# mathcom/G2Vec

Hardware: NVIDIA H100
Metric: cbow_context_windows_per_sec (higher is better)
Workload: dtype f32

## Files before the change

g2vec_b200/_capi.py:

```python
import ctypes
import os

from . import build as _build

_lib = None

_vp, _i32, _i64, _u32, _u64, _f32 = (ctypes.c_void_p, ctypes.c_int32, ctypes.c_int64, ctypes.c_uint32,
                                     ctypes.c_uint64, ctypes.c_float)

SIGNATURES = {
    "g2v_abi_version": (ctypes.c_int, []),
    "g2v_last_error": (ctypes.c_char_p, []),
    "g2v_device_info": (ctypes.c_int, [_vp, _vp, _vp, _vp]),
    "g2v_launch_count": (_i64, []),
    "g2v_walk_workspace_bytes": (ctypes.c_size_t, []),
    "g2v_walk_launch": (ctypes.c_int, [_vp, _vp, _vp, _i32, _i64, _i32, _u64, _u32, _i64, _i64, _i64,
                                       _vp, _vp, _vp, _vp]),
    "g2v_walk_packed_bytes": (ctypes.c_int, [_i32, _i64, _vp, _vp]),
    "g2v_walk_prepare": (ctypes.c_int, [_vp, _vp, _vp, _i32, _i64, _vp, _vp, _vp, _vp, _vp]),
    "g2v_walk_launch_packed": (ctypes.c_int, [_vp, _vp, _i32, _i32, _i64, _i32, _u64, _u32, _i64, _i64, _i64,
                                              _vp, _vp, _vp, _vp, _vp]),
    "g2v_walk_host": (ctypes.c_int, [_vp, _vp, _vp, _i32, _i64, _i32, _u64, _u32, _i64, _i64, _i64, _vp, _vp]),
    "g2v_cbow_fwdbwd": (ctypes.c_int, [_vp, _vp, _vp, _vp, _i64, _i64, _f32, _vp, _vp, _vp, _vp, _vp, _vp,
                                       _i32, _i32, _i32, _vp]),
    "g2v_cbow_fwdbwd_csc": (ctypes.c_int, [_vp, _vp, _vp, _vp, _i64, _f32, _vp, _vp, _vp, _vp, _vp, _vp, _vp, _vp,
                                           _vp, _i32, _i32, _i32, _vp]),
    "g2v_cbow_fwd_do": (ctypes.c_int, [_vp, _vp, _vp, _vp, _i64, _f32, _vp, _vp, _vp, _vp, _vp, _vp, _i32, _i32, _i32,
                                       _vp]),
    "g2v_cbow_lazy_adam": (ctypes.c_int, [_vp, _vp, _vp, _vp, _i64, _vp, _vp, _vp, _vp, _vp, _vp, _vp, _i32, _i32, _f32,
                                          _f32, _f32, _f32, _i32, _vp, _vp]),
    "g2v_cbow_det_workspace_bytes": (ctypes.c_size_t, [_i64, _i32]),
    "g2v_cbow_fwdbwd_csc_det": (ctypes.c_int, [_vp, _vp, _vp, _vp, _i64, _f32, _vp, _vp, _vp, _vp, _vp, _vp, _vp, _vp,
                                               _vp, _i32, _i32, _i32, _vp, _i32, _vp]),
    "g2v_cbow_fwd_do_det": (ctypes.c_int, [_vp, _vp, _vp, _vp, _i64, _f32, _vp, _vp, _vp, _vp, _vp, _vp, _i32, _i32,
                                           _i32, _vp, _i32, _vp]),
    "g2v_cbow_loop_tail_det": (ctypes.c_int, [_vp, _vp, _vp, _vp, _vp, _i64, _f32, _vp, _vp, _vp, _vp, _vp, _i32, _i32,
                                              _i32, _vp, _i32, _vp]),
    "g2v_cbow_batch_expand": (ctypes.c_int, [_vp, _vp, _vp, _vp, _i64, _vp, _vp, _i32, _i32, _i32, _vp]),
    "g2v_cbow_epoch_order": (ctypes.c_int, [_vp, _i64, _u64, _i32, _i64, _i64, _vp, _vp]),
    "g2v_cbow_batch_plan_workspace_bytes": (ctypes.c_size_t, [_i64, _i64, _i64, _i32]),
    "g2v_cbow_batch_plan": (ctypes.c_int, [_vp, _vp, _vp, _i64, _i64, _i64, _i32, _vp, _vp, _vp, _vp, _vp, _vp]),
    "g2v_cbow_update": (ctypes.c_int, [_vp, _vp, _vp, _vp, _vp, _vp, _vp, _vp, _i32, _i32, _i32, _f32, _f32,
                                       _f32, _f32, _i32, _vp, _vp]),
    "g2v_cbow_update_nvl": (ctypes.c_int, [_vp, _vp, _vp, _vp, _vp, _vp, _i64, _i32, _i32, _i32, _f32, _f32, _f32,
                                           _f32, _i32, _vp, _vp]),
    "g2v_cbow_adam_tick": (ctypes.c_int, [_vp, _f32, _f32, _f32, _vp]),
    "g2v_cbow_eval": (ctypes.c_int, [_vp, _vp, _vp, _vp, _i64, _i64, _vp, _vp, _vp, _i32, _i32, _i32, _vp]),
    "g2v_cbow_loop_init": (ctypes.c_int, [_vp, _i64, _i32, _vp]),
    "g2v_cbow_loop_attach": (ctypes.c_int, [_vp]),
    "g2v_cbow_loop_begin": (ctypes.c_int, [_vp, _vp, _vp, _vp, _i64, _vp]),
    "g2v_cbow_loop_tail": (ctypes.c_int, [_vp, _vp, _vp, _vp, _vp, _i64, _f32, _vp, _vp, _vp, _vp, _vp, _i32, _i32, _i32,
                                          _vp]),
    "g2v_cbow_loop_decide": (ctypes.c_int, [_vp, _vp, _vp, _vp]),
    "g2v_cbow_loop_decide_best": (ctypes.c_int, [_vp, _vp, _vp, _vp, _vp]),
    "g2v_cbow_loop_keep_best": (ctypes.c_int, [_vp, _vp, _vp, _i64, _vp]),
    "g2v_cbow_loop_counters_nvl": (ctypes.c_int, [_vp, _vp, _vp, _vp, _i32, _vp]),
    "g2v_cbow_slab_plan": (ctypes.c_int, [_i32, _i32, _vp]),
    "g2v_cbow_slab_workspace_bytes": (ctypes.c_size_t, [_i64, _i32, _i32]),
    "g2v_cbow_slab_setup": (ctypes.c_int, [_vp, _vp, _vp, _i64, _i64, _i32, _i32, _vp, _vp]),
    "g2v_cbow_fwdbwd_slabs": (ctypes.c_int, [_vp, _vp, _vp, _i64, _i64, _f32, _vp, _vp, _vp, _vp, _vp, _vp,
                                             _i32, _i32, _i32, _i32, _vp, _vp]),
    "g2v_cbow_eval_slabs": (ctypes.c_int, [_vp, _vp, _vp, _i64, _i64, _vp, _vp, _vp, _i32, _i32, _i32, _i32, _vp, _vp]),
    "g2v_cbow_step_host": (ctypes.c_int, [_vp, _vp, _vp, _i64, _i64, _vp, _vp, _vp, _vp, _vp, _vp, _i32, _i32,
                                          _i32, _i32, _f32, _f32, _f32, _f32, _i32, _vp, _vp]),
    "g2v_cbow_r1_prepare": (ctypes.c_int, [_vp, _vp, _vp, _i32, _i32, _vp]),
    "g2v_cbow_r1_windows": (ctypes.c_int, [_vp, _vp, _vp, _vp, _i64, _i64, _f32, _vp, _vp, _vp, _vp, _i32, _i32, _vp]),
    "g2v_cbow_r1_windows_csc": (ctypes.c_int, [_vp, _vp, _vp, _vp, _i64, _f32, _vp, _vp, _vp, _vp, _vp, _vp, _vp,
                                              _i32, _i32, _vp]),
    "g2v_cbow_r1_scratch_bytes": (ctypes.c_size_t, [_i32]),
    "g2v_cbow_r1_update": (ctypes.c_int, [_vp, _vp, _vp, _vp, _vp, _vp, _vp, _vp, _vp, _i32, _i32, _i32, _f32, _f32,
                                         _f32, _f32, _i32, _vp, _vp]),
    "g2v_pcc_zscore": (ctypes.c_int, [_vp, _i32, _i32, _vp, _vp]),
    "g2v_pcc_edge_weights": (ctypes.c_int, [_vp, _i32, _i32, _vp, _vp, _i64, _vp, _vp]),
    "g2v_paths_canonicalise": (ctypes.c_int, [_vp, _i64, _i32, _vp, _vp, _vp]),
    "g2v_paths_mark": (ctypes.c_int, [_vp, _vp, _vp, _vp, _i64, _i32, _vp, _vp]),
    "g2v_paths_set_workspace_bytes": (ctypes.c_size_t, [_i64]),
    "g2v_paths_set_select": (ctypes.c_int, [_vp, _vp, _vp, _vp, _i64, _i32, _vp, _vp, _vp, _vp]),
    "g2v_paths_set_emit": (ctypes.c_int, [_vp, _vp, _vp, _vp, _i64, _i32, _i32, _vp, _i64, _i64, _vp, _vp, _vp, _vp,
                                          _vp, _vp]),
    "g2v_test_l2_rows": (ctypes.c_int, [_vp, _vp, _vp, _i64, _i32, _i32, _vp, _vp]),
# ... 45 lines not shown
```

g2vec_b200/cbow.py:

```python
import math
import time

import numpy as np
import torch

from . import _capi


def split_indices(n, seed):
    perm = np.arange(n, dtype=np.int64)
    np.random.RandomState(seed).shuffle(perm)
    pivot = int(n * 0.8)
    return perm[:pivot], perm[pivot:]


def truncated_normal(shape, stddev, rng):
    x = rng.standard_normal(size=shape)
    bad = np.abs(x) > 2.0
    while bad.any():
        x[bad] = rng.standard_normal(size=int(bad.sum()))
        bad = np.abs(x) > 2.0
    return (x * stddev).astype(np.float32)


# ... 25 lines not shown
        self.device = dev

        def to(a, dt):
            if isinstance(a, torch.Tensor):
                return a.to(device=dev, dtype=dt).contiguous()
            return torch.from_numpy(np.ascontiguousarray(a)).to(device=dev, dtype=dt)

        self.rowptr = to(rowptr, torch.int32)
        self.gene = to(gene, torch.int32)
        self.label = to(label, torch.uint8)
        self.V, self.D = int(n_genes), int(hidden)
        n_flat = self.V * self.D + self.D
        self.nvl = None
        self.lazy = optimizer == "lazy_adam"
        self.det = bool(deterministic)
        self._det_ws = None
        self._lists, self._pending, self._dO = {}, None, None
        if algo == "rows" and nvl_group is not None:
            self.nvl = _nvl_setup(nvl_group, n_flat, dev)
        if algo == "rows":
            self.w_flat = self.nvl["w"] if self.nvl else torch.empty(n_flat, dtype=torch.float32, device=dev)
            self.W_ih = self.w_flat[:self.V * self.D].view(self.V, self.D)
            self.W_ho = self.w_flat[self.V * self.D:]
            self.W_ih.copy_(to(W_ih0, torch.float32).reshape(self.V, self.D))
            self.W_ho.copy_(to(W_ho0, torch.float32).reshape(self.D))
        else:
            self.W_ih = to(W_ih0, torch.float32).reshape(self.V, self.D).clone()
            self.W_ho = to(W_ho0, torch.float32).reshape(self.D).clone()
        self.opt = {"adam": _capi.OPT_ADAM_TF1, "sgd": _capi.OPT_SGD, "lazy_adam": _capi.OPT_ADAM_TF1}[optimizer]
        self.reduce = {"sum": _capi.REDUCE_SUM, "mean": _capi.REDUCE_MEAN}[reduce]
        self.lr, self.beta1, self.beta2, self.eps = float(lr), float(beta1), float(beta2), float(eps)
        z = lambda *s: torch.zeros(*s, dtype=torch.float32, device=dev)
        self.algo = algo
        if self.lazy:
            self.g_ih, self.g_ho = None, z(self.D)
            self.g_flat = self.g_ho
            self.s = self.c = None
        elif algo == "rows":
            self.g_flat = self.nvl["g"].zero_() if self.nvl else z(n_flat)
            self.g_ih = self.g_flat[:self.V * self.D].view(self.V, self.D)
            self.g_ho = self.g_flat[self.V * self.D:]
            self.s = self.c = None
        else:
            self.g_ih = None
            self.g_ho = z(int(self.lib.g2v_cbow_r1_scratch_bytes(self.D)) // 4)
            self.s, self.c = z(self.V), z(self.V)
        self.m_flat = self.v_flat = None
        if self.opt == _capi.OPT_ADAM_TF1 and algo == "rows":
            self.m_flat, self.v_flat = z(n_flat), z(n_flat)
            vd = self.V * self.D
            self.m_ih, self.v_ih = self.m_flat[:vd].view(self.V, self.D), self.v_flat[:vd].view(self.V, self.D)
            self.m_ho, self.v_ho = self.m_flat[vd:], self.v_flat[vd:]
        elif self.opt == _capi.OPT_ADAM_TF1:
            self.m_ih, self.v_ih, self.m_ho, self.v_ho = z(self.V, self.D), z(self.V, self.D), z(self.D), z(self.D)
        else:
            self.m_ih = self.v_ih = self.m_ho = self.v_ho = None
        self.acc = torch.zeros(6, dtype=torch.int64, device=dev)
        self.t = 0
        self.hyper = torch.tensor([1.0, 1.0, 0.0, 0.0], dtype=torch.float32, device=dev)
        if algo == "rank1":
            self._launch("g2v_cbow_r1_prepare", self.W_ih.data_ptr(), self.W_ho.data_ptr(), self.s.data_ptr(), self.V,
                         self.D)

    def _launch(self, name, *args):
        rc = getattr(self.lib, name)(*args, self._stream())
        if rc:
# ... 184 lines not shown
        if self.algo == "rank1":
            self._launch("g2v_cbow_r1_update", self.W_ih.data_ptr(), self.W_ho.data_ptr(), self._ptr(self.m_ih),
                         self._ptr(self.v_ih), self._ptr(self.m_ho), self._ptr(self.v_ho), self.c.data_ptr(),
                         self.g_ho.data_ptr(), self.s.data_ptr(), self.V, self.D, self.opt, self.lr, self.beta1,
                         self.beta2, self.eps, self.t, adev)
            return
        if self.nvl:
            nv = self.nvl
            nv["hg"].barrier(channel=0)
            self._launch("g2v_cbow_update_nvl", nv["hg"].buffer_ptrs_dev, nv["hw"].buffer_ptrs_dev, nv["g_mc"],
                         nv["w_mc"], self._ptr(self.m_flat), self._ptr(self.v_flat), self.V * self.D + self.D,
                         nv["rank"], nv["world"], self.opt, self.lr, self.beta1, self.beta2, self.eps, self.t, adev)
            nv["hg"].barrier(channel=1)
            return
        self._launch("g2v_cbow_update", self.W_ih.data_ptr(), self.W_ho.data_ptr(), self._ptr(self.m_ih),
                     self._ptr(self.v_ih), self._ptr(self.m_ho), self._ptr(self.v_ho), self.g_ih.data_ptr(),
                     self.g_ho.data_ptr(), self.V, self.D, self.opt, self.lr, self.beta1, self.beta2, self.eps, self.t,
                     adev)

    def evaluate(self, win, slot, win_begin=0, n_win=None):
        lo = int(win_begin)
        n = int((win.shape[0] - win_begin) if n_win is None else n_win)
        rec = self.prepared(win)
        r = choose_route(self.algo, False, False, rec, lo, n)
        acc = self.acc.data_ptr() + 8 * slot
        if r in ("r1", "r1_csc"):
            self._launch("g2v_cbow_r1_windows", self.rowptr.data_ptr(), self.gene.data_ptr(), self.label.data_ptr(),
                         self._ptr(win), lo, n, 0.0, self.s.data_ptr(), 0, 0, acc, self.V, self.reduce)
        elif r == "slabs":
            self._launch("g2v_cbow_eval_slabs", self.gene.data_ptr(), self.label.data_ptr(), self._ptr(win), lo, n,
                         self.W_ih.data_ptr(), self.W_ho.data_ptr(), acc, self.V, self.D, self.reduce, self._n_slabs,
                         rec.slabs[(lo, n)].data_ptr())
        else:
            self._launch("g2v_cbow_eval", self.rowptr.data_ptr(), self.gene.data_ptr(), self.label.data_ptr(),
                         self._ptr(win), lo, n, self.W_ih.data_ptr(), self.W_ho.data_ptr(), acc, self.V, self.D,
                         self.reduce)

    def loss_sum(self, acc_host):
        return float(acc_host[:1].view(torch.float64)[0])


def check_config(algo, optimizer, deterministic, several_gpus=False, batch=0, reshuffle=False, patience=1):
    if isinstance(patience, bool) or not isinstance(patience, (int, np.integer)) or patience < 1:
        raise ValueError("patience must be an int >= 1 (the number of bad epochs in a row that stops the run)")
    if algo not in ("rows", "rank1"):
        raise ValueError("algo must be 'rows' (gather/scatter of embedding rows) or 'rank1' (collapsed)")
    if reshuffle and batch <= 0:
        raise ValueError("reshuffle=True needs mini-batches (batch > 0)")
    if deterministic and several_gpus:
        raise ValueError("deterministic=True runs on one GPU only")
    if deterministic and algo == "rank1" and batch > 0:
        raise ValueError("deterministic=True with algo='rank1' needs a full batch: rank1's mini-batch c uses atomics")
    if optimizer == "lazy_adam" and algo != "rows":
        raise ValueError("optimizer='lazy_adam' needs algo='rows' (rank1 keeps s = W_ih.W_ho, which every W_ho step "
                         "changes for every gene)")
    if optimizer == "lazy_adam" and several_gpus:
        raise ValueError("optimizer='lazy_adam' runs on one GPU only")


class _WindowList:

    def __init__(self, win, n):
        self.win, self.n = win, n
        self.cscptr = self.pos = self.dO = None
        self.slabs = {}
        self.plan, self.B, self.brp = None, 0, None

    def whole(self, win_begin, n):
        return self.cscptr is not None and win_begin == 0 and n == self.n
# ... 503 lines not shown
```

g2vec_b200/csrc/g2v_cbow.cu:

```cuda
#include "g2v_cbow_common.cuh"

namespace g2v {

constexpr int kRowsEval = 0, kRowsScatter = 1, kRowsCsc = 2;

template <int VEC, int MODE>
__global__ void __launch_bounds__(kCbowWarps * 32)
cbow_rows_kernel(const int32_t *__restrict__ rowptr, const int32_t *__restrict__ gene,
                 const uint8_t *__restrict__ label, const int32_t *__restrict__ win,
                 int64_t win_begin, int64_t n_win, float inv_n, const float *__restrict__ W_ih,
                 const float *__restrict__ W_ho, float *__restrict__ g_ih, float *__restrict__ g_ho,
                 double *__restrict__ loss_sum, unsigned long long *__restrict__ n_correct,
                 int32_t reduce_mean, const int32_t *__restrict__ skip, float *__restrict__ dO_pos,
                 const int32_t *__restrict__ carried) {
    G2V_SKIP_IF_STOPPED(skip);
    G2V_SKIP_IF_STOPPED(carried);
    constexpr bool BACKWARD = MODE != kRowsEval;
    constexpr int D = 128 * VEC;
    constexpr int D4 = D / 4;
    constexpr int UNR = 8 / VEC;
    __shared__ float sh_gho[BACKWARD ? D : 1];
    __shared__ CtaAcc sh_acc;
    const int lane = threadIdx.x & 31, warp = threadIdx.x >> 5;
    if (BACKWARD) for (int i = threadIdx.x; i < D; i += blockDim.x) sh_gho[i] = 0.f;
    if (threadIdx.x == 0) { sh_acc.loss = 0.0; sh_acc.correct = 0ull; }
    __syncthreads();

    const float4 *__restrict__ W4 = reinterpret_cast<const float4 *>(W_ih);
    float4 who[VEC], gho[VEC];
#pragma unroll
    for (int v = 0; v < VEC; ++v) {
        who[v] = ldg4(reinterpret_cast<const float4 *>(W_ho) + v * 32 + lane);
        gho[v] = make_float4(0.f, 0.f, 0.f, 0.f);
    }
    unsigned correct_acc = 0;
    float loss_acc = 0.f;

    const int64_t warps_total = (int64_t)gridDim.x * kCbowWarps;
    for (int64_t i = (int64_t)blockIdx.x * kCbowWarps + warp; i < n_win; i += warps_total) {
        const int64_t n = win ? (int64_t)__ldg(win + win_begin + i) : win_begin + i;
        const int32_t b = __ldg(rowptr + n), e = __ldg(rowptr + n + 1);
        const float y = (float)__ldg(label + n);
        float4 h[VEC];
#pragma unroll
        for (int v = 0; v < VEC; ++v) h[v] = make_float4(0.f, 0.f, 0.f, 0.f);
        for (int32_t base = b; base < e; base += 32) {
            const int cnt = min(32, e - base);
            const int32_t g = (lane < cnt) ? __ldg(gene + base + lane) : 0;
            for (int k = 0; k < cnt; k += UNR) {
                float4 r[UNR][VEC];
#pragma unroll
                for (int u = 0; u < UNR; ++u) {
                    const int32_t gk = __shfl_sync(0xffffffffu, g, (k + u) & 31);
                    const float4 *row = W4 + (size_t)gk * D4 + lane;
#pragma unroll
                    for (int v = 0; v < VEC; ++v)
                        r[u][v] = (k + u < cnt) ? ldg4(row + v * 32) : make_float4(0.f, 0.f, 0.f, 0.f);
                }
#pragma unroll
                for (int u = 0; u < UNR; ++u)
#pragma unroll
                    for (int v = 0; v < VEC; ++v) {
                        h[v].x += r[u][v].x; h[v].y += r[u][v].y; h[v].z += r[u][v].z; h[v].w += r[u][v].w;
                    }
            }
        }
        const float scale = (reduce_mean && e > b) ? 1.f / (float)(e - b) : 1.f;
        float part = 0.f;
#pragma unroll
        for (int v = 0; v < VEC; ++v) {
            if (reduce_mean) { h[v].x *= scale; h[v].y *= scale; h[v].z *= scale; h[v].w *= scale; }
            part += h[v].x * who[v].x + h[v].y * who[v].y + h[v].z * who[v].z + h[v].w * who[v].w;
        }
        const float o = warp_sum(part);
        if (lane == 0) {
            correct_acc += ((o > 0.f) == (y != 0.f)) ? 1u : 0u;
            if (BACKWARD) loss_acc += fmaxf(o, 0.f) - o * y + log1pf(expf(-fabsf(o)));
        }
        if (MODE == kRowsCsc) {
            const float dO = (sigmoid_stable(o) - y) * inv_n;
#pragma unroll
            for (int v = 0; v < VEC; ++v) {
                gho[v].x += h[v].x * dO; gho[v].y += h[v].y * dO; gho[v].z += h[v].z * dO; gho[v].w += h[v].w * dO;
            }
            if (lane == 0) dO_pos[i] = dO * scale;
        } else if (MODE == kRowsScatter) {
            const float dO = (sigmoid_stable(o) - y) * inv_n;
            float4 gv[VEC];
#pragma unroll
            for (int v = 0; v < VEC; ++v) {
                gho[v].x += h[v].x * dO; gho[v].y += h[v].y * dO; gho[v].z += h[v].z * dO; gho[v].w += h[v].w * dO;
                const float s = dO * scale;
                gv[v] = make_float4(who[v].x * s, who[v].y * s, who[v].z * s, who[v].w * s);
            }
            for (int32_t base = b; base < e; base += 32) {
                const int cnt = min(32, e - base);
                const int32_t g = (lane < cnt) ? __ldg(gene + base + lane) : 0;
                for (int k = 0; k < cnt; ++k) {
                    const int32_t gk = __shfl_sync(0xffffffffu, g, k);
                    float *dst = g_ih + (size_t)gk * D + lane * 4;
#pragma unroll
                    for (int v = 0; v < VEC; ++v) red_add4(dst + v * 128, gv[v]);
                }
            }
        }
    }
    cta_epilogue<VEC, BACKWARD, true>(sh_gho, sh_acc, gho, loss_acc, correct_acc, lane, g_ho, loss_sum, n_correct);
}

template <bool BACKWARD>
__global__ void __launch_bounds__(kCbowWarps * 32)
cbow_rows_generic_kernel(const int32_t *__restrict__ rowptr, const int32_t *__restrict__ gene,
                         const uint8_t *__restrict__ label, const int32_t *__restrict__ win,
                         int64_t win_begin, int64_t n_win, float inv_n, const float *__restrict__ W_ih,
                         const float *__restrict__ W_ho, float *__restrict__ g_ih,
                         float *__restrict__ g_ho, double *__restrict__ loss_sum,
                         unsigned long long *__restrict__ n_correct, int32_t D, int32_t reduce_mean,
                         const int32_t *__restrict__ skip, float *__restrict__ dO_pos,
                         const int32_t *__restrict__ carried) {
    G2V_SKIP_IF_STOPPED(skip);
    G2V_SKIP_IF_STOPPED(carried);
    extern __shared__ float shf[];
    __shared__ CtaAcc sh_acc;
    const int lane = threadIdx.x & 31, warp = threadIdx.x >> 5;
    float *h = shf + (size_t)warp * 2 * D;
    float *gho = h + D;
    for (int d = lane; d < D; d += 32) gho[d] = 0.f;
    if (threadIdx.x == 0) { sh_acc.loss = 0.0; sh_acc.correct = 0ull; }
    __syncthreads();
    float loss_acc = 0.f;
    unsigned correct_acc = 0;
    const int64_t warps_total = (int64_t)gridDim.x * kCbowWarps;
    for (int64_t i = (int64_t)blockIdx.x * kCbowWarps + warp; i < n_win; i += warps_total) {
        const int64_t n = win ? (int64_t)__ldg(win + win_begin + i) : win_begin + i;
        const int32_t b = __ldg(rowptr + n), e = __ldg(rowptr + n + 1);
        const float y = (float)__ldg(label + n);
        for (int d = lane; d < D; d += 32) h[d] = 0.f;
        for (int32_t j = b; j < e; ++j) {
            const float *row = W_ih + (size_t)__ldg(gene + j) * D;
            for (int d = lane; d < D; d += 32) h[d] += __ldg(row + d);
        }
        const float scale = (reduce_mean && e > b) ? 1.f / (float)(e - b) : 1.f;
        float part = 0.f;
        for (int d = lane; d < D; d += 32) {
            if (reduce_mean) h[d] *= scale;
            part += h[d] * __ldg(W_ho + d);
        }
        const float o = warp_sum(part);
        if (lane == 0) {
            correct_acc += ((o > 0.f) == (y != 0.f)) ? 1u : 0u;
            if (BACKWARD) loss_acc += fmaxf(o, 0.f) - o * y + log1pf(expf(-fabsf(o)));
        }
        if (BACKWARD) {
            const float dO = (sigmoid_stable(o) - y) * inv_n;
            for (int d = lane; d < D; d += 32) gho[d] += h[d] * dO;
            const float s = dO * scale;
            if (dO_pos) {
                if (lane == 0) dO_pos[i] = s;
                continue;
            }
            for (int32_t j = b; j < e; ++j) {
                float *dst = g_ih + (size_t)__ldg(gene + j) * D;
                for (int d = lane; d < D; d += 32) atomicAdd(dst + d, __ldg(W_ho + d) * s);
            }
        }
    }
    if (BACKWARD) for (int d = lane; d < D; d += 32) atomicAdd(g_ho + d, gho[d]);
    if (lane == 0) {
        if (BACKWARD) atomicAdd(&sh_acc.loss, (double)loss_acc);
        atomicAdd(&sh_acc.correct, (unsigned long long)correct_acc);
    }
    __syncthreads();
    if (threadIdx.x == 0) {
        if (BACKWARD && loss_sum) atomicAdd(loss_sum, sh_acc.loss);
        if (n_correct) atomicAdd(n_correct, sh_acc.correct);
    }
}

__global__ void __launch_bounds__(kCbowWarps * 32)
cbow_csc_expand_kernel(const int32_t *__restrict__ cscptr, const int32_t *__restrict__ csc_pos,
                       const float *__restrict__ dO_pos, const float *__restrict__ W_ho, float *__restrict__ g_ih,
                       int32_t V, int32_t D, const int32_t *__restrict__ skip) {
    G2V_SKIP_IF_STOPPED(skip);
    const int lane = threadIdx.x & 31;
    const int64_t warp = (int64_t)blockIdx.x * kCbowWarps + (threadIdx.x >> 5);
    const int64_t nwarps = (int64_t)gridDim.x * kCbowWarps;
    for (int64_t g = warp; g < V; g += nwarps) {
        const int32_t b = __ldg(cscptr + g), e = __ldg(cscptr + g + 1);
        if (b == e) continue;
        const float c = csc_segment_sum(csc_pos, dO_pos, b, e, lane);
        float *row = g_ih + (size_t)g * D;
        if ((D & 3) == 0) {
            float4 *r4 = reinterpret_cast<float4 *>(row);
            for (int k = lane; k < (D >> 2); k += 32) {
                const float4 w = ldg4(reinterpret_cast<const float4 *>(W_ho) + k);
                float4 a = r4[k];
                a.x += c * w.x; a.y += c * w.y; a.z += c * w.z; a.w += c * w.w;
                r4[k] = a;
            }
        } else {
            for (int d = lane; d < D; d += 32) row[d] += c * __ldg(W_ho + d);
        }
    }
}

constexpr int kDetTile = 64;
constexpr int kDetSumWarps = 32;

// ... 771 lines not shown
    if (rc) return rc;
    loop_carry_kernel<<<1, 1, 0, st>>>(reinterpret_cast<long long *>(ctl), reinterpret_cast<long long *>(acc));
    G2V_CUDA_OK(cudaGetLastError());
    count_launch();
    return 0;
}

extern "C" int g2v_cbow_batch_expand(const int32_t *rows, const int32_t *segptr, const int32_t *pos, const float *dO,
                                     int64_t n_rows, const float *W_ho, float *g_ih, int32_t V, int32_t D,
                                     int32_t max_ctas, void *stream) {
    G2V_REQUIRE(V > 0 && D > 0 && n_rows >= 0 && n_rows <= V && max_ctas >= 0,
                "g2v_cbow_batch_expand: bad sizes (V=%d D=%d n_rows=%lld max_ctas=%d)", V, D, (long long)n_rows, max_ctas);
    G2V_REQUIRE(n_rows == 0 || (rows && segptr && pos && dO && W_ho && g_ih), "g2v_cbow_batch_expand: null pointer");
    if (n_rows == 0) return 0;
    int grid = 0, rc;
    if ((rc = det_grid((const void *)cbow_batch_expand_kernel, 0, n_rows, max_ctas, &grid))) return rc;
    cbow_batch_expand_kernel<<<grid, kCbowWarps * 32, 0, (cudaStream_t)stream>>>(rows, segptr, pos, dO, n_rows, W_ho,
                                                                                  g_ih, D, loop_skip_flag());
    G2V_CUDA_OK(cudaGetLastError());
    count_launch();
    return 0;
}

extern "C" int g2v_cbow_eval(const int32_t *rowptr, const int32_t *gene, const uint8_t *label,
                             const int32_t *win, int64_t win_begin, int64_t n_win, const float *W_ih,
                             const float *W_ho, int64_t *n_correct, int32_t V, int32_t D, int32_t reduce,
                             void *stream) {
    G2V_REQUIRE(V > 0 && D > 0 && n_win >= 0 && win_begin >= 0, "g2v_cbow_eval: bad sizes");
    G2V_REQUIRE(rowptr && label && W_ih && W_ho && n_correct, "g2v_cbow_eval: null pointer");
    G2V_REQUIRE(reduce == G2V_REDUCE_SUM || reduce == G2V_REDUCE_MEAN, "g2v_cbow_eval: unknown reduce %d", reduce);
    if (n_win == 0) return 0;
    return launch_rows<false>(rowptr, gene, label, win, win_begin, n_win, 0.f, W_ih, W_ho, nullptr, nullptr,
                              nullptr, n_correct, D, reduce, (cudaStream_t)stream);
}

__global__ void adam_tick_kernel(float *state, float lr, float beta1, float beta2, const int32_t *skip) {
    G2V_SKIP_IF_STOPPED(skip);
    const float b1p = state[0] * beta1, b2p = state[1] * beta2;
    state[0] = b1p; state[1] = b2p;
    state[2] = lr * sqrtf(1.f - b2p) / (1.f - b1p);
}

extern "C" int g2v_cbow_adam_tick(float *state, float lr, float beta1, float beta2, void *stream) {
    G2V_REQUIRE(state != nullptr, "g2v_cbow_adam_tick: null pointer");
    adam_tick_kernel<<<1, 1, 0, (cudaStream_t)stream>>>(state, lr, beta1, beta2, loop_skip_flag());
    G2V_CUDA_OK(cudaGetLastError());
    count_launch();
    return 0;
}

extern "C" int g2v_cbow_update(float *W_ih, float *W_ho, float *m_ih, float *v_ih, float *m_ho, float *v_ho,
                               float *g_ih, float *g_ho, int32_t V, int32_t D, int32_t optimizer, float lr,
                               float beta1, float beta2, float eps, int32_t t, const float *alpha_dev,
                               void *stream) {
    G2V_REQUIRE(V > 0 && D > 0 && (t >= 1 || alpha_dev), "g2v_cbow_update: bad sizes (V=%d D=%d t=%d)", V, D, t);
    G2V_REQUIRE(W_ih && W_ho && g_ih && g_ho, "g2v_cbow_update: null pointer");
    G2V_REQUIRE(optimizer == G2V_OPT_ADAM_TF1 || optimizer == G2V_OPT_SGD, "g2v_cbow_update: unknown optimizer %d", optimizer);
    G2V_REQUIRE(optimizer == G2V_OPT_SGD || (m_ih && v_ih && m_ho && v_ho), "g2v_cbow_update: Adam needs m/v buffers");
    DeviceProps dp;
    if (device_props(&dp)) return 1;
    const int64_t n = (int64_t)V * D;
    int64_t blocks = (n / 4 + 255) / 256;
    const int64_t cap = (int64_t)dp.sm_count * 8;
    if (blocks > cap) blocks = cap;
    if (blocks < 1) blocks = 1;
    cudaStream_t st = (cudaStream_t)stream;
// ... 131 lines not shown
```

g2vec_b200/csrc/g2v_cbow_common.cuh:

```cuda
#pragma once
#include "g2v_common.cuh"

namespace g2v {

constexpr int kCbowWarps = 8;

__device__ __forceinline__ float4 ldg4(const float4 *p) { return __ldg(p); }
__device__ __forceinline__ void red_add4(float *p, float4 v) {
    asm volatile("red.global.add.v4.f32 [%0], {%1, %2, %3, %4};" ::"l"(p), "f"(v.x), "f"(v.y), "f"(v.z),
                 "f"(v.w)
                 : "memory");
}
__device__ __forceinline__ float sigmoid_stable(float x) {
    if (x >= 0.f) { const float z = expf(-x); return 1.f / (1.f + z); }
    const float z = expf(x);
    return z / (1.f + z);
}

__device__ __forceinline__ void adam1(float &w, float &m, float &v, float g, float alpha, float omb1,
                                      float omb2, float eps) {
    m += (g - m) * omb1;
    v += (g * g - v) * omb2;
    w -= (m * alpha) / (sqrtf(v) + eps);
}
// ... 4 lines not shown
    return lr * sqrtf(1.f - b2p) / (1.f - b1p);
}

struct CtaAcc {
    double loss;
    unsigned long long correct;
};

template <int VEC, bool TRAIN, bool ACTIVE>
__device__ __forceinline__ void cta_epilogue(float *sh_gho, CtaAcc &sh_acc, const float4 (&gho)[VEC], float loss_acc,
                                             unsigned correct_acc, int lane, float *__restrict__ g_ho,
                                             double *__restrict__ loss_sum, unsigned long long *__restrict__ n_correct) {
    constexpr int D = 128 * VEC;
    if (TRAIN && ACTIVE) {
#pragma unroll
        for (int v = 0; v < VEC; ++v) {
            float *p = sh_gho + (v * 32 + lane) * 4;
            atomicAdd(p + 0, gho[v].x); atomicAdd(p + 1, gho[v].y);
            atomicAdd(p + 2, gho[v].z); atomicAdd(p + 3, gho[v].w);
        }
    }
    if (ACTIVE && lane == 0) {
        if (TRAIN) atomicAdd(&sh_acc.loss, (double)loss_acc);
        atomicAdd(&sh_acc.correct, (unsigned long long)correct_acc);
    }
    __syncthreads();
    if (TRAIN && ACTIVE) for (int i = threadIdx.x; i < D; i += blockDim.x) atomicAdd(g_ho + i, sh_gho[i]);
    if (ACTIVE && threadIdx.x == 0) {
        if (TRAIN && loss_sum) atomicAdd(loss_sum, sh_acc.loss);
        if (n_correct) atomicAdd(n_correct, sh_acc.correct);
    }
}

int rows_grid(const void *kernel, size_t smem, int64_t n_items, int *grid_out);

}
```

g2vec_b200/csrc/g2v_cbow_rank1.cu:

```cuda
#include "g2v_cbow_common.cuh"

namespace g2v {

__global__ void __launch_bounds__(kCbowWarps * 32)
r1_prepare_kernel(const float *__restrict__ W_ih, const float *__restrict__ W_ho, float *__restrict__ s,
                  int32_t V, int32_t D, const int32_t *__restrict__ skip) {
    G2V_SKIP_IF_STOPPED(skip);
    const int lane = threadIdx.x & 31;
    const int64_t warp = (int64_t)blockIdx.x * kCbowWarps + (threadIdx.x >> 5);
    const int64_t nwarps = (int64_t)gridDim.x * kCbowWarps;
    const bool vec4 = (D & 3) == 0;
    for (int64_t g = warp; g < V; g += nwarps) {
        const float *row = W_ih + (size_t)g * D;
        float part = 0.f;
        if (vec4) {
            const float4 *r4 = reinterpret_cast<const float4 *>(row);
            const float4 *h4 = reinterpret_cast<const float4 *>(W_ho);
            for (int i = lane; i < (D >> 2); i += 32) {
                const float4 a = __ldg(r4 + i), b = __ldg(h4 + i);
                part += a.x * b.x + a.y * b.y + a.z * b.z + a.w * b.w;
            }
        } else {
            for (int d = lane; d < D; d += 32) part += __ldg(row + d) * __ldg(W_ho + d);
        }
        part = warp_sum(part);
        if (lane == 0) s[g] = part;
    }
}

template <int MODE>
__global__ void __launch_bounds__(kCbowWarps * 32)
r1_windows_kernel(const int32_t *__restrict__ rowptr, const int32_t *__restrict__ gene,
                  const uint8_t *__restrict__ label, const int32_t *__restrict__ win, int64_t win_begin,
                  int64_t n_win, float inv_n, const float *__restrict__ s, float *__restrict__ c,
                  double *__restrict__ loss_sum, unsigned long long *__restrict__ n_correct,
                  int32_t reduce_mean, const int32_t *__restrict__ skip) {
    G2V_SKIP_IF_STOPPED(skip);
    constexpr bool BACKWARD = MODE != 0;
    __shared__ CtaAcc sh;
    const int lane = threadIdx.x & 31, warp = threadIdx.x >> 5;
    const int sub = lane & 7, slot = lane >> 3;
    if (threadIdx.x == 0) { sh.loss = 0.0; sh.correct = 0ull; }
    __syncthreads();
    float loss_acc = 0.f;
    unsigned correct_acc = 0;
    const int64_t stride = (int64_t)gridDim.x * kCbowWarps * 4;
    for (int64_t base = ((int64_t)blockIdx.x * kCbowWarps + warp) * 4; base < n_win; base += stride) {
        const int64_t i = base + slot;
        const bool active = i < n_win;
        int32_t b = 0, e = 0;
        float y = 0.f;
        if (active) {
            const int64_t n = win ? (int64_t)__ldg(win + win_begin + i) : win_begin + i;
            b = __ldg(rowptr + n); e = __ldg(rowptr + n + 1);
            y = (float)__ldg(label + n);
        }
        float part = 0.f;
        for (int32_t j = b + sub; j < e; j += 8) part += __ldg(s + __ldg(gene + j));
        part += __shfl_xor_sync(0xffffffffu, part, 4);
// ... 129 lines not shown
r1_update_ho_kernel(float *__restrict__ W_ho, float *__restrict__ m, float *__restrict__ v,
                    const float *__restrict__ g_part, int32_t n_part, int32_t D, float alpha_host, float omb1,
                    float omb2, float eps, const float *__restrict__ alpha_dev, const int32_t *__restrict__ skip) {
    G2V_SKIP_IF_STOPPED(skip);
    const float alpha = alpha_dev ? __ldg(alpha_dev + 2) : alpha_host;
    __shared__ float sh[32][33];
    const int lane = threadIdx.x & 31, slice = threadIdx.x >> 5;
    const int i = blockIdx.x * 32 + lane;
    float a = 0.f;
    if (i < D)
        for (int p = slice; p < n_part; p += 32) a += g_part[(size_t)p * D + i];
    sh[slice][lane] = a;
    __syncthreads();
    if (slice == 0 && i < D) {
        float g = 0.f;
#pragma unroll
        for (int q = 0; q < 32; ++q) g += sh[q][lane];
        float w = W_ho[i];
        if (OPT == G2V_OPT_ADAM_TF1) {
            float mm = m[i], vv = v[i];
            adam1(w, mm, vv, g, alpha, omb1, omb2, eps);
            m[i] = mm; v[i] = vv;
        } else {
            w -= alpha * g;
        }
        W_ho[i] = w;
    }
}

}

using namespace g2v;

extern "C" int g2v_cbow_r1_prepare(const float *W_ih, const float *W_ho, float *s, int32_t V, int32_t D,
                                   void *stream) {
    G2V_REQUIRE(V > 0 && D > 0 && W_ih && W_ho && s, "g2v_cbow_r1_prepare: bad arguments");
    int grid = 0, rc;
    if ((rc = rows_grid((const void *)r1_prepare_kernel, 0, V, &grid))) return rc;
    r1_prepare_kernel<<<grid, kCbowWarps * 32, 0, (cudaStream_t)stream>>>(W_ih, W_ho, s, V, D, loop_skip_flag());
    G2V_CUDA_OK(cudaGetLastError());
    count_launch();
    return 0;
}

extern "C" int g2v_cbow_r1_windows(const int32_t *rowptr, const int32_t *gene, const uint8_t *label,
                                   const int32_t *win, int64_t win_begin, int64_t n_win, float inv_n_total,
                                   const float *s, float *c, double *loss_sum, int64_t *n_correct, int32_t V,
                                   int32_t reduce, void *stream) {
    G2V_REQUIRE(V > 0 && n_win >= 0 && win_begin >= 0, "g2v_cbow_r1_windows: bad sizes");
    G2V_REQUIRE(rowptr && label && s, "g2v_cbow_r1_windows: null pointer");
    G2V_REQUIRE(reduce == G2V_REDUCE_SUM || reduce == G2V_REDUCE_MEAN, "g2v_cbow_r1_windows: unknown reduce %d", reduce);
    if (n_win == 0) return 0;
    unsigned long long *nc = reinterpret_cast<unsigned long long *>(n_correct);
    int grid = 0, rc;
    cudaStream_t st = (cudaStream_t)stream;
    if (c) {
        if ((rc = rows_grid((const void *)r1_windows_kernel<1>, 0, (n_win + 3) / 4, &grid))) return rc;
        r1_windows_kernel<1><<<grid, kCbowWarps * 32, 0, st>>>(rowptr, gene, label, win, win_begin, n_win,
                                                              inv_n_total, s, c, loss_sum, nc, reduce, loop_skip_flag());
    } else {
        if ((rc = rows_grid((const void *)r1_windows_kernel<0>, 0, (n_win + 3) / 4, &grid))) return rc;
        r1_windows_kernel<0><<<grid, kCbowWarps * 32, 0, st>>>(rowptr, gene, label, win, win_begin, n_win, 0.f,
                                                              s, nullptr, nullptr, nc, reduce, loop_skip_flag());
    }
    G2V_CUDA_OK(cudaGetLastError());
    count_launch();
    return 0;
}

extern "C" int g2v_cbow_r1_windows_csc(const int32_t *rowptr, const int32_t *gene, const uint8_t *label,
                                       const int32_t *win, int64_t n_win, float inv_n_total, const float *s,
                                       const int32_t *cscptr, const int32_t *csc_pos, float *dO, float *c,
                                       double *loss_sum, int64_t *n_correct, int32_t V, int32_t reduce,
                                       void *stream) {
    G2V_REQUIRE(V > 0 && n_win >= 0, "g2v_cbow_r1_windows_csc: bad sizes");
// ... 77 lines not shown
```

include/g2vec_b200.h:

```cpp
#ifndef G2VEC_B200_H
#define G2VEC_B200_H

#include <stddef.h>
#include <stdint.h>

#ifdef __cplusplus
extern "C" {
#endif

#define G2V_ABI_VERSION 2

#define G2V_OPT_ADAM_TF1 0
#define G2V_OPT_SGD 1

#define G2V_REDUCE_SUM 0
#define G2V_REDUCE_MEAN 1

int g2v_abi_version(void);
const char *g2v_last_error(void);

int g2v_device_info(int32_t *sm_count, int32_t *cc_major, int32_t *cc_minor, int64_t *l2_bytes);
int64_t g2v_launch_count(void);

size_t g2v_walk_workspace_bytes(void);
// ... 46 lines not shown
                        int64_t n_win, float inv_n_total, const float *W_ih, const float *W_ho, float *dO, float *g_ho,
                        double *loss_sum, int64_t *n_correct, int32_t V, int32_t D, int32_t reduce, void *workspace,
                        int32_t max_ctas, void *stream);
int g2v_cbow_loop_tail_det(int64_t *ctl, const int32_t *rowptr, const int32_t *gene, const uint8_t *label,
                           const int32_t *win, int64_t n_win, float inv_n_total, const float *W_ih, const float *W_ho,
                           float *dO, float *g_ho, int64_t *acc, int32_t V, int32_t D, int32_t reduce, void *workspace,
                           int32_t max_ctas, void *stream);
int g2v_cbow_batch_expand(const int32_t *rows, const int32_t *segptr, const int32_t *pos, const float *dO,
                          int64_t n_rows, const float *W_ho, float *g_ih, int32_t V, int32_t D, int32_t max_ctas,
                          void *stream);

int g2v_cbow_epoch_order(const int32_t *tr, int64_t n, uint64_t seed, int32_t epoch, int64_t rank, int64_t world,
                         int32_t *out, void *stream);
size_t g2v_cbow_batch_plan_workspace_bytes(int64_t n_win, int64_t nnz, int64_t B, int32_t V);
int g2v_cbow_batch_plan(const int32_t *rowptr, const int32_t *gene, const int32_t *win, int64_t n_win, int64_t nnz,
                        int64_t B, int32_t V, int32_t *rows, int32_t *segptr, int32_t *pos, int32_t *batch_rowptr,
                        void *workspace, void *stream);

int g2v_cbow_update(float *W_ih, float *W_ho, float *m_ih, float *v_ih, float *m_ho, float *v_ho,
                    float *g_ih, float *g_ho, int32_t V, int32_t D, int32_t optimizer, float lr,
                    float beta1, float beta2, float eps, int32_t t, const float *alpha_dev, void *stream);

int g2v_cbow_update_nvl(float *const *g_ptrs_dev, float *const *w_ptrs_dev, float *g_multicast, float *w_multicast,
                        float *m_flat, float *v_flat, int64_t n, int32_t rank, int32_t world, int32_t optimizer,
                        float lr, float beta1, float beta2, float eps, int32_t t, const float *alpha_dev, void *stream);

int g2v_cbow_adam_tick(float *state, float lr, float beta1, float beta2, void *stream);

int g2v_cbow_eval(const int32_t *rowptr, const int32_t *gene, const uint8_t *label,
                  const int32_t *win, int64_t win_begin, int64_t n_win, const float *W_ih,
                  const float *W_ho, int64_t *n_correct, int32_t V, int32_t D, int32_t reduce,
                  void *stream);

int g2v_cbow_loop_init(int64_t *ctl, int64_t max_steps, int32_t early_stop, void *stream);
int g2v_cbow_loop_attach(const int64_t *ctl);
int g2v_cbow_loop_begin(const int64_t *ctl, int64_t *acc, const float *W_ih, float *snapshot, int64_t n, void *stream);
int g2v_cbow_loop_tail(int64_t *ctl, const int32_t *rowptr, const int32_t *gene, const uint8_t *label,
                       const int32_t *win, int64_t n_win, float inv_n_total, const float *W_ih, const float *W_ho,
                       float *dO, float *g_ho, int64_t *acc, int32_t V, int32_t D, int32_t reduce, void *stream);
int g2v_cbow_loop_decide(int64_t *ctl, const int64_t *acc, int64_t *hist, void *stream);
int g2v_cbow_loop_decide_best(int64_t *ctl, int64_t *best, const int64_t *acc, int64_t *hist, void *stream);
int g2v_cbow_loop_keep_best(const int64_t *best, const float *W_ih, float *result, int64_t n, void *stream);
int g2v_cbow_loop_counters_nvl(const int64_t *ctl, const int64_t *acc, int64_t *const *hist_ptrs_dev,
                               int64_t *hist_multicast, int32_t world, void *stream);

int g2v_cbow_slab_plan(int32_t V, int32_t D, int32_t *n_slabs);
size_t g2v_cbow_slab_workspace_bytes(int64_t n_win, int32_t D, int32_t n_slabs);
int g2v_cbow_slab_setup(const int32_t *rowptr, const int32_t *gene, const int32_t *win, int64_t win_begin,
                        int64_t n_win, int32_t V, int32_t n_slabs, void *workspace, void *stream);
int g2v_cbow_fwdbwd_slabs(const int32_t *gene, const uint8_t *label, const int32_t *win, int64_t win_begin,
                          int64_t n_win, float inv_n_total, const float *W_ih, const float *W_ho, float *g_ih,
                          float *g_ho, double *loss_sum, int64_t *n_correct, int32_t V, int32_t D, int32_t reduce,
                          int32_t n_slabs, void *workspace, void *stream);
int g2v_cbow_eval_slabs(const int32_t *gene, const uint8_t *label, const int32_t *win, int64_t win_begin,
                        int64_t n_win, const float *W_ih, const float *W_ho, int64_t *n_correct, int32_t V,
                        int32_t D, int32_t reduce, int32_t n_slabs, void *workspace, void *stream);

int g2v_cbow_step_host(const int32_t *rowptr, const int32_t *gene, const uint8_t *label,
                       int64_t n_win, int64_t nnz, float *W_ih, float *W_ho, float *m_ih,
                       float *v_ih, float *m_ho, float *v_ho, int32_t V, int32_t D,
                       int32_t optimizer, int32_t reduce, float lr, float beta1, float beta2,
                       float eps, int32_t t, double *loss_sum, int64_t *n_correct);

int g2v_cbow_r1_prepare(const float *W_ih, const float *W_ho, float *s, int32_t V, int32_t D,
                        void *stream);
int g2v_cbow_r1_windows(const int32_t *rowptr, const int32_t *gene, const uint8_t *label,
// ... 40 lines not shown
```

Baseline: 153.3 million.

## Certify eval predictions via precomputed per-gene logits with error bounds

```diff
diff --git a/g2vec_b200/_capi.py b/g2vec_b200/_capi.py
--- a/g2vec_b200/_capi.py
+++ b/g2vec_b200/_capi.py
@@ -46,6 +46,8 @@
                                            _f32, _i32, _vp, _vp]),
     "g2v_cbow_adam_tick": (ctypes.c_int, [_vp, _f32, _f32, _f32, _vp]),
     "g2v_cbow_eval": (ctypes.c_int, [_vp, _vp, _vp, _vp, _i64, _i64, _vp, _vp, _vp, _i32, _i32, _i32, _vp]),
+    "g2v_cbow_eval_certified": (ctypes.c_int, [_vp, _vp, _vp, _vp, _i64, _i64, _vp, _vp, _vp, _vp, _vp, _i32, _i32,
+                                               _i32, _i32, _vp]),
     "g2v_cbow_loop_init": (ctypes.c_int, [_vp, _i64, _i32, _vp]),
     "g2v_cbow_loop_attach": (ctypes.c_int, [_vp]),
     "g2v_cbow_loop_begin": (ctypes.c_int, [_vp, _vp, _vp, _vp, _i64, _vp]),
diff --git a/g2vec_b200/cbow.py b/g2vec_b200/cbow.py
--- a/g2vec_b200/cbow.py
+++ b/g2vec_b200/cbow.py
@@ -81,6 +81,7 @@
         self.lr, self.beta1, self.beta2, self.eps = float(lr), float(beta1), float(beta2), float(eps)
         z = lambda *s: torch.zeros(*s, dtype=torch.float32, device=dev)
         self.algo = algo
+        self.st = z(2 * self.V) if algo == "rows" else None
         if self.lazy:
             self.g_ih, self.g_ho = None, z(self.D)
             self.g_flat = self.g_ho
@@ -331,9 +332,9 @@
                          self.W_ih.data_ptr(), self.W_ho.data_ptr(), acc, self.V, self.D, self.reduce, self._n_slabs,
                          rec.slabs[(lo, n)].data_ptr())
         else:
-            self._launch("g2v_cbow_eval", self.rowptr.data_ptr(), self.gene.data_ptr(), self.label.data_ptr(),
-                         self._ptr(win), lo, n, self.W_ih.data_ptr(), self.W_ho.data_ptr(), acc, self.V, self.D,
-                         self.reduce)
+            self._launch("g2v_cbow_eval_certified", self.rowptr.data_ptr(), self.gene.data_ptr(),
+                         self.label.data_ptr(), self._ptr(win), lo, n, self.W_ih.data_ptr(), self.W_ho.data_ptr(),
+                         self.st.data_ptr(), acc, None, self.V, self.D, self.reduce, 0)
 
     def loss_sum(self, acc_host):
         return float(acc_host[:1].view(torch.float64)[0])
diff --git a/g2vec_b200/csrc/g2v_cbow.cu b/g2vec_b200/csrc/g2v_cbow.cu
--- a/g2vec_b200/csrc/g2v_cbow.cu
+++ b/g2vec_b200/csrc/g2v_cbow.cu
@@ -17,8 +17,6 @@
     G2V_SKIP_IF_STOPPED(carried);
     constexpr bool BACKWARD = MODE != kRowsEval;
     constexpr int D = 128 * VEC;
-    constexpr int D4 = D / 4;
-    constexpr int UNR = 8 / VEC;
     __shared__ float sh_gho[BACKWARD ? D : 1];
     __shared__ CtaAcc sh_acc;
     const int lane = threadIdx.x & 31, warp = threadIdx.x >> 5;
@@ -42,37 +40,8 @@
         const int32_t b = __ldg(rowptr + n), e = __ldg(rowptr + n + 1);
         const float y = (float)__ldg(label + n);
         float4 h[VEC];
-#pragma unroll
-        for (int v = 0; v < VEC; ++v) h[v] = make_float4(0.f, 0.f, 0.f, 0.f);
-        for (int32_t base = b; base < e; base += 32) {
-            const int cnt = min(32, e - base);
-            const int32_t g = (lane < cnt) ? __ldg(gene + base + lane) : 0;
-            for (int k = 0; k < cnt; k += UNR) {
-                float4 r[UNR][VEC];
-#pragma unroll
-                for (int u = 0; u < UNR; ++u) {
-                    const int32_t gk = __shfl_sync(0xffffffffu, g, (k + u) & 31);
-                    const float4 *row = W4 + (size_t)gk * D4 + lane;
-#pragma unroll
-                    for (int v = 0; v < VEC; ++v)
-                        r[u][v] = (k + u < cnt) ? ldg4(row + v * 32) : make_float4(0.f, 0.f, 0.f, 0.f);
-                }
-#pragma unroll
-                for (int u = 0; u < UNR; ++u)
-#pragma unroll
-                    for (int v = 0; v < VEC; ++v) {
-                        h[v].x += r[u][v].x; h[v].y += r[u][v].y; h[v].z += r[u][v].z; h[v].w += r[u][v].w;
-                    }
-            }
-        }
-        const float scale = (reduce_mean && e > b) ? 1.f / (float)(e - b) : 1.f;
-        float part = 0.f;
-#pragma unroll
-        for (int v = 0; v < VEC; ++v) {
-            if (reduce_mean) { h[v].x *= scale; h[v].y *= scale; h[v].z *= scale; h[v].w *= scale; }
-            part += h[v].x * who[v].x + h[v].y * who[v].y + h[v].z * who[v].z + h[v].w * who[v].w;
-        }
-        const float o = warp_sum(part);
+        float scale;
+        const float o = rows_logit<VEC>(gene, W4, b, e, lane, reduce_mean, who, h, scale);
         if (lane == 0) {
             correct_acc += ((o > 0.f) == (y != 0.f)) ? 1u : 0u;
             if (BACKWARD) loss_acc += fmaxf(o, 0.f) - o * y + log1pf(expf(-fabsf(o)));
@@ -135,18 +104,8 @@
         const int64_t n = win ? (int64_t)__ldg(win + win_begin + i) : win_begin + i;
         const int32_t b = __ldg(rowptr + n), e = __ldg(rowptr + n + 1);
         const float y = (float)__ldg(label + n);
-        for (int d = lane; d < D; d += 32) h[d] = 0.f;
-        for (int32_t j = b; j < e; ++j) {
-            const float *row = W_ih + (size_t)__ldg(gene + j) * D;
-            for (int d = lane; d < D; d += 32) h[d] += __ldg(row + d);
-        }
-        const float scale = (reduce_mean && e > b) ? 1.f / (float)(e - b) : 1.f;
-        float part = 0.f;
-        for (int d = lane; d < D; d += 32) {
-            if (reduce_mean) h[d] *= scale;
-            part += h[d] * __ldg(W_ho + d);
-        }
-        const float o = warp_sum(part);
+        float scale;
+        const float o = rows_generic_logit(gene, W_ih, W_ho, b, e, lane, D, reduce_mean, h, scale);
         if (lane == 0) {
             correct_acc += ((o > 0.f) == (y != 0.f)) ? 1u : 0u;
             if (BACKWARD) loss_acc += fmaxf(o, 0.f) - o * y + log1pf(expf(-fabsf(o)));
@@ -174,6 +133,107 @@
     if (threadIdx.x == 0) {
         if (BACKWARD && loss_sum) atomicAdd(loss_sum, sh_acc.loss);
         if (n_correct) atomicAdd(n_correct, sh_acc.correct);
+    }
+}
+
+__device__ __forceinline__ float certified_tau(float T, float scale, int32_t l, int32_t D, float A) {
+    const int64_t k = (int64_t)l + D + 16;
+    if (!(T <= 0x1p126f) || k > (1 << 22)) return __int_as_float(0x7f800000);
+    const float rel = __fmul_rn(__fmul_rn((float)k, 0x1p-21f), scale);
+    const float abs_ = __fmul_rn(__fadd_rn((float)(((int64_t)l + 3) * D), A), 0x1p-145f);
+    return __fadd_rn(__fmul_rn(rel, T), abs_);
+}
+
+template <int VEC>
+__global__ void __launch_bounds__(kCbowWarps * 32)
+cbow_eval_certified_kernel(const int32_t *__restrict__ rowptr, const int32_t *__restrict__ gene,
+                           const uint8_t *__restrict__ label, const int32_t *__restrict__ win, int64_t win_begin,
+                           int64_t n_win, const float *__restrict__ W_ih, const float *__restrict__ W_ho,
+                           const float2 *__restrict__ st, unsigned long long *__restrict__ n_correct,
+                           unsigned long long *__restrict__ n_gathered, int32_t D, int32_t reduce_mean,
+                           int32_t force_gather, const int32_t *__restrict__ skip) {
+    G2V_SKIP_IF_STOPPED(skip);
+    constexpr int NV = VEC > 0 ? VEC : 1;
+    extern __shared__ float shf[];
+    __shared__ unsigned long long sh_cnt[2];
+    const int lane = threadIdx.x & 31, warp = threadIdx.x >> 5;
+    const int sub = lane & 7, slot = lane >> 3;
+    if (threadIdx.x < 2) sh_cnt[threadIdx.x] = 0ull;
+    __syncthreads();
+    const float4 *__restrict__ W4 = reinterpret_cast<const float4 *>(W_ih);
+    float4 who[NV];
+    if (VEC > 0) {
+#pragma unroll
+        for (int v = 0; v < NV; ++v) who[v] = ldg4(reinterpret_cast<const float4 *>(W_ho) + v * 32 + lane);
+    }
+    float *h_generic = shf + (size_t)warp * D;
+    float A = 0.f;
+    if (VEC == 0) {
+        for (int d = lane; d < D; d += 32) A += fabsf(__ldg(W_ho + d));
+        A = warp_sum(A);
+    }
+    unsigned correct_acc = 0, gathered_acc = 0;
+    const int64_t stride = (int64_t)gridDim.x * kCbowWarps * 4;
+    for (int64_t base = ((int64_t)blockIdx.x * kCbowWarps + warp) * 4; base < n_win; base += stride) {
+        const int64_t i = base + slot;
+        const bool active = i < n_win;
+        int32_t b = 0, e = 0;
+        float y = 0.f;
+        if (active) {
+            const int64_t n = win ? (int64_t)__ldg(win + win_begin + i) : win_begin + i;
+            b = __ldg(rowptr + n); e = __ldg(rowptr + n + 1);
+            y = (float)__ldg(label + n);
+        }
+        float ps = 0.f, pt = 0.f;
+        for (int32_t j = b + sub; j < e; j += 8) {
+            const float2 q = __ldg(st + __ldg(gene + j));
+            ps += q.x; pt += q.y;
+        }
+#pragma unroll
+        for (int o = 4; o > 0; o >>= 1) {
+            ps += __shfl_xor_sync(0xffffffffu, ps, o);
+            pt += __shfl_xor_sync(0xffffffffu, pt, o);
+        }
+        if (VEC > 0) {
+            A = 0.f;
+#pragma unroll
+            for (int v = 0; v < NV; ++v)
+                A += (fabsf(who[v].x) + fabsf(who[v].y)) + (fabsf(who[v].z) + fabsf(who[v].w));
+            A = warp_sum(A);
+        }
+        const float scale = (reduce_mean && e > b) ? 1.f / (float)(e - b) : 1.f;
+        const float o1 = ps * scale;
+        const bool decided = !force_gather && fabsf(o1) <= 0x1.fffffep127f
+                             && fabsf(o1) > certified_tau(pt, scale, e - b, D, A);
+        if (active && sub == 0 && decided) correct_acc += ((o1 > 0.f) == (y != 0.f)) ? 1u : 0u;
+        unsigned todo = __ballot_sync(0xffffffffu, active && sub == 0 && !decided);
+        while (todo) {
+            const int src = __ffs(todo) - 1;
+            todo &= todo - 1;
+            const int32_t wb = __shfl_sync(0xffffffffu, b, src), we = __shfl_sync(0xffffffffu, e, src);
+            const float wy = __shfl_sync(0xffffffffu, y, src);
+            float wscale, o;
+            if (VEC > 0) {
+                float4 h[NV];
+                o = rows_logit<NV>(gene, W4, wb, we, lane, reduce_mean, who, h, wscale);
+            } else {
+                o = rows_generic_logit(gene, W_ih, W_ho, wb, we, lane, D, reduce_mean, h_generic, wscale);
+            }
+            if (lane == 0) {
+                correct_acc += ((o > 0.f) == (wy != 0.f)) ? 1u : 0u;
+                ++gathered_acc;
+            }
+        }
+    }
+    correct_acc = __reduce_add_sync(0xffffffffu, correct_acc);
+    if (lane == 0) {
+        atomicAdd(&sh_cnt[0], (unsigned long long)correct_acc);
+        atomicAdd(&sh_cnt[1], (unsigned long long)gathered_acc);
+    }
+    __syncthreads();
+    if (threadIdx.x == 0) {
+        atomicAdd(n_correct, sh_cnt[0]);
+        if (n_gathered) atomicAdd(n_gathered, sh_cnt[1]);
     }
 }
 
@@ -1011,6 +1071,44 @@
     if (n_win == 0) return 0;
     return launch_rows<false>(rowptr, gene, label, win, win_begin, n_win, 0.f, W_ih, W_ho, nullptr, nullptr,
                               nullptr, n_correct, D, reduce, (cudaStream_t)stream);
+}
+
+extern "C" int g2v_cbow_eval_certified(const int32_t *rowptr, const int32_t *gene, const uint8_t *label,
+                                       const int32_t *win, int64_t win_begin, int64_t n_win, const float *W_ih,
+                                       const float *W_ho, float *st, int64_t *n_correct, int64_t *n_gathered,
+                                       int32_t V, int32_t D, int32_t reduce, int32_t force_gather, void *stream) {
+    G2V_REQUIRE(V > 0 && D > 0 && n_win >= 0 && win_begin >= 0, "g2v_cbow_eval_certified: bad sizes");
+    G2V_REQUIRE(rowptr && label && W_ih && W_ho && st && n_correct, "g2v_cbow_eval_certified: null pointer");
+    G2V_REQUIRE(reduce == G2V_REDUCE_SUM || reduce == G2V_REDUCE_MEAN, "g2v_cbow_eval_certified: unknown reduce %d",
+                reduce);
+    if (n_win == 0) return 0;
+    cudaStream_t s = (cudaStream_t)stream;
+    const bool generic = D != 128 && D != 256 && D != 512;
+    const size_t smem = generic ? (size_t)kCbowWarps * D * sizeof(float) : 0;
+    if (generic) {
+        DeviceProps dp;
+        if (device_props(&dp)) return 1;
+        cudaFuncAttributes fa;
+        G2V_CUDA_OK(cudaFuncGetAttributes(&fa, cbow_rows_generic_kernel<false>));
+        G2V_REQUIRE((size_t)kCbowWarps * 2 * D * sizeof(float) + fa.sharedSizeBytes <= (size_t)dp.max_smem_optin,
+                    "sizeHiddenlayer %d too large for the generic kernel", D);
+        G2V_CUDA_OK(cudaFuncSetAttribute(cbow_eval_certified_kernel<0>, cudaFuncAttributeMaxDynamicSharedMemorySize,
+                                         (int)smem));
+    }
+    int rc = launch_r1_prepare(W_ih, W_ho, st, V, D, true, s);
+    if (rc) return rc;
+    auto kern = D == 128 ? cbow_eval_certified_kernel<1> : D == 256 ? cbow_eval_certified_kernel<2>
+              : D == 512 ? cbow_eval_certified_kernel<4> : cbow_eval_certified_kernel<0>;
+    int grid = 0;
+    if ((rc = rows_grid((const void *)kern, smem, (n_win + 3) / 4, &grid))) return rc;
+    kern<<<grid, kCbowWarps * 32, smem, s>>>(rowptr, gene, label, win, win_begin, n_win, W_ih, W_ho,
+                                            reinterpret_cast<const float2 *>(st),
+                                            reinterpret_cast<unsigned long long *>(n_correct),
+                                            reinterpret_cast<unsigned long long *>(n_gathered), D,
+                                            reduce == G2V_REDUCE_MEAN, force_gather, loop_skip_flag());
+    G2V_CUDA_OK(cudaGetLastError());
+    count_launch();
+    return 0;
 }
 
 __global__ void adam_tick_kernel(float *state, float lr, float beta1, float beta2, const int32_t *skip) {
diff --git a/g2vec_b200/csrc/g2v_cbow_common.cuh b/g2vec_b200/csrc/g2v_cbow_common.cuh
--- a/g2vec_b200/csrc/g2v_cbow_common.cuh
+++ b/g2vec_b200/csrc/g2v_cbow_common.cuh
@@ -60,6 +60,65 @@
     }
 }
 
+template <int VEC>
+__device__ __forceinline__ float rows_logit(const int32_t *__restrict__ gene, const float4 *__restrict__ W4, int32_t b,
+                                            int32_t e, int lane, int32_t reduce_mean, const float4 (&who)[VEC],
+                                            float4 (&h)[VEC], float &scale) {
+    constexpr int D4 = 32 * VEC;
+    constexpr int UNR = 8 / VEC;
+#pragma unroll
+    for (int v = 0; v < VEC; ++v) h[v] = make_float4(0.f, 0.f, 0.f, 0.f);
+    for (int32_t base = b; base < e; base += 32) {
+        const int cnt = min(32, e - base);
+        const int32_t g = (lane < cnt) ? __ldg(gene + base + lane) : 0;
+        for (int k = 0; k < cnt; k += UNR) {
+            float4 r[UNR][VEC];
+#pragma unroll
+            for (int u = 0; u < UNR; ++u) {
+                const int32_t gk = __shfl_sync(0xffffffffu, g, (k + u) & 31);
+                const float4 *row = W4 + (size_t)gk * D4 + lane;
+#pragma unroll
+                for (int v = 0; v < VEC; ++v)
+                    r[u][v] = (k + u < cnt) ? ldg4(row + v * 32) : make_float4(0.f, 0.f, 0.f, 0.f);
+            }
+#pragma unroll
+            for (int u = 0; u < UNR; ++u)
+#pragma unroll
+                for (int v = 0; v < VEC; ++v) {
+                    h[v].x += r[u][v].x; h[v].y += r[u][v].y; h[v].z += r[u][v].z; h[v].w += r[u][v].w;
+                }
+        }
+    }
+    scale = (reduce_mean && e > b) ? 1.f / (float)(e - b) : 1.f;
+    float part = 0.f;
+#pragma unroll
+    for (int v = 0; v < VEC; ++v) {
+        if (reduce_mean) { h[v].x *= scale; h[v].y *= scale; h[v].z *= scale; h[v].w *= scale; }
+        part += h[v].x * who[v].x + h[v].y * who[v].y + h[v].z * who[v].z + h[v].w * who[v].w;
+    }
+    return warp_sum(part);
+}
+
+__device__ __forceinline__ float rows_generic_logit(const int32_t *__restrict__ gene, const float *__restrict__ W_ih,
+                                                    const float *__restrict__ W_ho, int32_t b, int32_t e, int lane,
+                                                    int32_t D, int32_t reduce_mean, float *h, float &scale) {
+    for (int d = lane; d < D; d += 32) h[d] = 0.f;
+    for (int32_t j = b; j < e; ++j) {
+        const float *row = W_ih + (size_t)__ldg(gene + j) * D;
+        for (int d = lane; d < D; d += 32) h[d] += __ldg(row + d);
+    }
+    scale = (reduce_mean && e > b) ? 1.f / (float)(e - b) : 1.f;
+    float part = 0.f;
+    for (int d = lane; d < D; d += 32) {
+        if (reduce_mean) h[d] *= scale;
+        part += h[d] * __ldg(W_ho + d);
+    }
+    return warp_sum(part);
+}
+
 int rows_grid(const void *kernel, size_t smem, int64_t n_items, int *grid_out);
 
+int launch_r1_prepare(const float *W_ih, const float *W_ho, float *s, int32_t V, int32_t D, bool with_t,
+                      cudaStream_t stream);
+
 }
diff --git a/g2vec_b200/csrc/g2v_cbow_rank1.cu b/g2vec_b200/csrc/g2v_cbow_rank1.cu
--- a/g2vec_b200/csrc/g2v_cbow_rank1.cu
+++ b/g2vec_b200/csrc/g2v_cbow_rank1.cu
@@ -2,6 +2,7 @@
 
 namespace g2v {
 
+template <bool WITH_T>
 __global__ void __launch_bounds__(kCbowWarps * 32)
 r1_prepare_kernel(const float *__restrict__ W_ih, const float *__restrict__ W_ho, float *__restrict__ s,
                   int32_t V, int32_t D, const int32_t *__restrict__ skip) {
@@ -12,19 +13,38 @@
     const bool vec4 = (D & 3) == 0;
     for (int64_t g = warp; g < V; g += nwarps) {
         const float *row = W_ih + (size_t)g * D;
-        float part = 0.f;
+        float part = 0.f, tpart = 0.f;
+        bool big = false;
         if (vec4) {
             const float4 *r4 = reinterpret_cast<const float4 *>(row);
             const float4 *h4 = reinterpret_cast<const float4 *>(W_ho);
             for (int i = lane; i < (D >> 2); i += 32) {
                 const float4 a = __ldg(r4 + i), b = __ldg(h4 + i);
                 part += a.x * b.x + a.y * b.y + a.z * b.z + a.w * b.w;
+                if (WITH_T) {
+                    tpart += fabsf(__fmul_rn(a.x, b.x)) + fabsf(__fmul_rn(a.y, b.y)) + fabsf(__fmul_rn(a.z, b.z))
+                             + fabsf(__fmul_rn(a.w, b.w));
+                    big |= fmaxf(fmaxf(fabsf(a.x), fabsf(a.y)), fmaxf(fabsf(a.z), fabsf(a.w))) > 0x1p64f;
+                }
             }
         } else {
-            for (int d = lane; d < D; d += 32) part += __ldg(row + d) * __ldg(W_ho + d);
+            for (int d = lane; d < D; d += 32) {
+                const float a = __ldg(row + d), b = __ldg(W_ho + d);
+                part += a * b;
+                if (WITH_T) {
+                    tpart += fabsf(__fmul_rn(a, b));
+                    big |= fabsf(a) > 0x1p64f;
+                }
+            }
         }
         part = warp_sum(part);
-        if (lane == 0) s[g] = part;
+        if (WITH_T) {
+            tpart = warp_sum(tpart);
+            if (__any_sync(0xffffffffu, big)) tpart = __int_as_float(0x7f800000);
+            if (lane == 0) reinterpret_cast<float2 *>(s)[g] = make_float2(part, tpart);
+        } else if (lane == 0) {
+            s[g] = part;
+        }
     }
 }
 
@@ -220,15 +240,26 @@
 
 using namespace g2v;
 
+namespace g2v {
+int launch_r1_prepare(const float *W_ih, const float *W_ho, float *s, int32_t V, int32_t D, bool with_t,
+                      cudaStream_t stream) {
+    const void *kern = with_t ? (const void *)r1_prepare_kernel<true> : (const void *)r1_prepare_kernel<false>;
+    int grid = 0, rc;
+    if ((rc = rows_grid(kern, 0, V, &grid))) return rc;
+    if (with_t)
+        r1_prepare_kernel<true><<<grid, kCbowWarps * 32, 0, stream>>>(W_ih, W_ho, s, V, D, loop_skip_flag());
+    else
+        r1_prepare_kernel<false><<<grid, kCbowWarps * 32, 0, stream>>>(W_ih, W_ho, s, V, D, loop_skip_flag());
+    G2V_CUDA_OK(cudaGetLastError());
+    count_launch();
+    return 0;
+}
+}
+
 extern "C" int g2v_cbow_r1_prepare(const float *W_ih, const float *W_ho, float *s, int32_t V, int32_t D,
                                    void *stream) {
     G2V_REQUIRE(V > 0 && D > 0 && W_ih && W_ho && s, "g2v_cbow_r1_prepare: bad arguments");
-    int grid = 0, rc;
-    if ((rc = rows_grid((const void *)r1_prepare_kernel, 0, V, &grid))) return rc;
-    r1_prepare_kernel<<<grid, kCbowWarps * 32, 0, (cudaStream_t)stream>>>(W_ih, W_ho, s, V, D, loop_skip_flag());
-    G2V_CUDA_OK(cudaGetLastError());
-    count_launch();
-    return 0;
+    return launch_r1_prepare(W_ih, W_ho, s, V, D, false, (cudaStream_t)stream);
 }
 
 extern "C" int g2v_cbow_r1_windows(const int32_t *rowptr, const int32_t *gene, const uint8_t *label,
diff --git a/include/g2vec_b200.h b/include/g2vec_b200.h
--- a/include/g2vec_b200.h
+++ b/include/g2vec_b200.h
@@ -102,6 +102,11 @@
                   const float *W_ho, int64_t *n_correct, int32_t V, int32_t D, int32_t reduce,
                   void *stream);
 
+int g2v_cbow_eval_certified(const int32_t *rowptr, const int32_t *gene, const uint8_t *label,
+                            const int32_t *win, int64_t win_begin, int64_t n_win, const float *W_ih,
+                            const float *W_ho, float *st, int64_t *n_correct, int64_t *n_gathered, int32_t V,
+                            int32_t D, int32_t reduce, int32_t force_gather, void *stream);
+
 int g2v_cbow_loop_init(int64_t *ctl, int64_t max_steps, int32_t early_stop, void *stream);
 int g2v_cbow_loop_attach(const int64_t *ctl);
 int g2v_cbow_loop_begin(const int64_t *ctl, int64_t *acc, const float *W_ih, float *snapshot, int64_t n, void *stream);
```

After: 176.9 million, median of 6. 15.4% higher.
